# maniac-mc/maniac-mc

Measured on AMD Instinct MI355X. Metric: MC moves/sec, higher is better.
Workload: dtype f64

## Files before the change

### maniac_mc_amd/csrc/mgpu_kernels_pair.h

```cpp
#ifndef MGPU_KERNELS_PAIR_H
#define MGPU_KERNELS_PAIR_H

#include "mgpu_kernels_common.h"

namespace mgpu {

template <int NS, bool ORDERED, bool TRI, bool FUSED, bool FASTW, bool SC1OUT = false>
__device__ __forceinline__ void pair_sweep_item(
    const Topo &tp, const BoxDev &bx, const double *__restrict__ pos, const int *__restrict__ nmol,
    const double *__restrict__ res_q, const int *__restrict__ res_atype, const double2 *__restrict__ pair_tab,
    const char *__restrict__ s_coul, const double2 *__restrict__ s_pair, double *__restrict__ w_site, int *__restrict__ w_sty,
    const PairItem it, const double *__restrict__ cand_sites, int site_stride, int split, int nsplit, int lane,
    double2 *__restrict__ partials, int w) {
    static_assert(!FUSED || (NS > 0 && !ORDERED && !TRI), "the fused old + new sweep is a register-site, unordered, orthorhombic path");
    static_assert(!FASTW || (NS > 0 && !ORDERED && !TRI), "the two-instruction fold is a register-site, unordered, orthorhombic path");
    constexpr int NTY = NS > 0 ? NS : 1;
    constexpr int NST = FUSED ? 2 : 1;
    constexpr int NREG = NTY * NST;
    const int nt = tp.n_types;
    [[maybe_unused]] const char *coul_adj = coul_tab_adjusted(s_coul, bx.coul_idx_base);
    {
        const double *px = pos + (size_t)it.replica * 3 * tp.n_cap_atoms;
        const double *py = px + tp.n_cap_atoms, *pz = py + tp.n_cap_atoms;
        const int *nm_r = nmol + it.replica * tp.n_res;
        const int n1 = NS > 0 ? NS : tp.n1[it.t];
        constexpr bool ordered = ORDERED;

        auto load_site = [&](int a, double &x, double &y, double &z) {
            if (it.src < 0) {
                const int j = atom_slot(tp, it.t, it.m, a);
                x = px[j]; y = py[j]; z = pz[j];
            } else {
                const double *c = cand_sites + ((size_t)it.src * site_stride + a) * 3;
                x = c[0]; y = c[1]; z = c[2];
            }
        };
        double rx[NREG], ry[NREG], rz[NREG], rq[NTY];
        int rty[NTY];
        if constexpr (NS > 0) {
#pragma unroll
            for (int a = 0; a < NTY; ++a) {
                if constexpr (FUSED) {
                    const int j = atom_slot(tp, it.t, it.m, a);
                    rx[a] = px[j]; ry[a] = py[j]; rz[a] = pz[j];
                    const double *c = cand_sites + ((size_t)it.src * site_stride + a) * 3;
                    rx[NTY + a] = c[0]; ry[NTY + a] = c[1]; rz[NTY + a] = c[2];
                    asm volatile("" : "+v"(rx[NTY + a]), "+v"(ry[NTY + a]), "+v"(rz[NTY + a]));
                } else {
                    load_site(a, rx[a], ry[a], rz[a]);
                }
                rq[a] = res_q[it.t * tp.max_atom + a];
                rty[a] = res_atype[it.t * tp.max_atom + a];
                asm volatile("" : "+v"(rx[a]), "+v"(ry[a]), "+v"(rz[a]));
            }
        }

        double elj[NST], ec[NST];
#pragma unroll
        for (int st = 0; st < NST; ++st) { elj[st] = 0.0; ec[st] = 0.0; }
        for (int sb = 0; sb < n1; sb += kSiteChunk) {
            const int ns = NS > 0 ? NS : min(kSiteChunk, n1 - sb);
            if constexpr (NS == 0) {
                __builtin_amdgcn_fence(__ATOMIC_ACQ_REL, "wavefront");
                __builtin_amdgcn_wave_barrier();
                if (lane < ns) {
                    double x, y, z;
                    load_site(sb + lane, x, y, z);
                    w_site[lane * 4 + 0] = x; w_site[lane * 4 + 1] = y; w_site[lane * 4 + 2] = z;
                    w_site[lane * 4 + 3] = res_q[it.t * tp.max_atom + sb + lane];
                    w_sty[lane] = res_atype[it.t * tp.max_atom + sb + lane];
                }
                __builtin_amdgcn_fence(__ATOMIC_ACQ_REL, "wavefront");
                __builtin_amdgcn_wave_barrier();
            }
            for (int t2 = 0, plane_base = 0; t2 < tp.n_res; plane_base += tp.n1[t2], ++t2) {
                if (ordered && t2 < it.t) continue;
                const int nm = nm_r[t2], n2 = tp.n1[t2];
                if (nm == 0) continue;
                const bool same_t = (t2 == it.t) && (it.m >= 0);
                [[maybe_unused]] auto plane_sweep = [&](const double *pxp, const double *pyp, const double *pzp,
                                                        int nm, bool excl, int dummy_m, double qj, int tyj, int key) {
                    const int cpp = (nm + 63) >> 6;
                    const bool qj_on = fabs(qj) >= kErrorTol;
                    double e4[NTY], sg2[NTY], qq[NTY];
                    bool lj[NTY], c_on[NTY];
                    bool any_c = false, all_c = true, any_lj = false;
#pragma unroll
                    for (int s = 0; s < NTY; ++s) {
                        const double2 pt = pair_tab[rty[s] * nt + tyj];
                        e4[s] = pt.x; sg2[s] = pt.y;
                        lj[s] = pt.x != 0.0;
                        c_on[s] = qj_on && (fabs(rq[s]) >= kErrorTol);
                        qq[s] = c_on[s] ? rq[s] * qj : 0.0;
                        any_c = any_c || c_on[s]; all_c = all_c && c_on[s]; any_lj = any_lj || lj[s];
                    }
                    if (!(any_c || any_lj)) return;
                    int c = split - (key * cpp) % nsplit;
                    if (c < 0) c += nsplit;
                    if (c >= cpp) return;
                    auto is_special = [&](int cc) {
                        return ORDERED || (cc == cpp - 1 && (nm & 63) != 0) || (excl && cc == (it.m >> 6));
                    };
                    auto fetch = [&](int cc, bool special, double &x, double &y, double &z, bool &ok) {
                        int m2 = cc * 64 + lane;
                        ok = true;
                        if (special) {
                            asm volatile("" ::: "memory");
                            ok = m2 < nm;
                            if (excl) ok = ok && (ORDERED ? (m2 > it.m) : (m2 != it.m));
                            m2 = ok ? m2 : dummy_m;
                        }
                        const unsigned ob = (unsigned)m2 * 8u;
                        x = *reinterpret_cast<const double *>(reinterpret_cast<const char *>(pxp) + ob);
                        y = *reinterpret_cast<const double *>(reinterpret_cast<const char *>(pyp) + ob);
                        z = *reinterpret_cast<const double *>(reinterpret_cast<const char *>(pzp) + ob);
                    };
                    double acc[NREG];
#pragma unroll
                    for (int s = 0; s < NREG; ++s) acc[s] = 0.0;
                    auto sweep_plane = [&](auto all_tag) {
                        constexpr bool ALL_C = decltype(all_tag)::value;
                        auto unit = [&](double xj, double yj, double zj, double wq, bool valid) {
                            const double rc2l = valid ? bx.rc2 : -1.0;
                            double r2[NREG], g[NREG];
                            unsigned sh_min = ~0u;
                            if constexpr (TRI) {
                                bool ok = bx.tri_lower != 0;
                                if (ok) {
#pragma unroll
                                    for (int s = 0; s < NREG; ++s) ok = image_r2_tri_lower(xj - rx[s], yj - ry[s], zj - rz[s], bx, r2[s]) && ok;
                                }
                                if (!__all(ok)) {
                                    asm volatile("" ::: "memory");
#pragma unroll
                                    for (int s = 0; s < NREG; ++s) r2[s] = image_r2_search27(xj - rx[s], yj - ry[s], zj - rz[s], bx.m);
                                }
                            } else {
#pragma unroll
                                for (int s = 0; s < NREG; ++s) {
                                    r2[s] = FASTW ? image_r2_fast(xj - rx[s], yj - ry[s], zj - rz[s], bx)
                                                  : image_r2<false>(xj - rx[s], yj - ry[s], zj - rz[s], bx);
                                }
                            }
#pragma unroll
                            for (int s = 0; s < NREG; ++s) {
                                if (!ALL_C && !c_on[s % NTY]) { g[s] = 0.0; continue; }
                                unsigned sh;
                                g[s] = coul_lds(r2[s], coul_adj, bx.coul_idx_far, sh);
                                sh_min = min(sh_min, sh);
                            }
                            if (sh_min < (unsigned)bx.coul_idx_base) {
#pragma unroll
                                for (int s = 0; s < NREG; ++s)
                                    if ((ALL_C || c_on[s % NTY]) && r2[s] < kCoulSlowBelow) g[s] = coul_slow(r2[s], bx.alpha, ORDERED);
                            }
#pragma unroll
                            for (int s = 0; s < NREG; ++s)
                                if (ALL_C || c_on[s % NTY]) acc[s] = fma(wq, g[s], acc[s]);
                            if (any_lj) {
#pragma unroll
                                for (int s = 0; s < NREG; ++s) {
                                    if (!lj[s % NTY]) continue;
                                    const double s2 = sg2[s % NTY] * fast_rcp(r2[s]);
                                    const double s6 = s2 * s2 * s2;
                                    const double e = e4[s % NTY] * fma(s6, s6, -s6);
                                    elj[s / NTY] += (r2[s] < rc2l) ? e : 0.0;
                                }
                            }
                        };
                        double xj, yj, zj;
                        bool valid, special = is_special(c);
                        fetch(c, special, xj, yj, zj, valid);
                        for (; c < cpp; c += nsplit) {
                            double xn = xj, yn = yj, zn = zj;
                            bool vn = true;
                            const bool special_n = is_special(c + nsplit);
                            if (c + nsplit < cpp) fetch(c + nsplit, special_n, xn, yn, zn, vn);
                            unit(xj, yj, zj, valid ? 1.0 : 0.0, valid);
                            xj = xn; yj = yn; zj = zn; valid = vn; special = special_n;
                        }
                    };
                    if (all_c) sweep_plane(std::true_type{});
                    else sweep_plane(std::false_type{});
#pragma unroll
                    for (int s = 0; s < NREG; ++s) ec[s / NTY] = fma(qq[s % NTY], acc[s], ec[s / NTY]);
                };
                if (!tp.site_major[t2]) {
                    if constexpr (NS > 0) {
                        const int cap2 = tp.cap[t2], seg2 = tp.seg_off[t2];
                        int dummy_m = 0;
                        if (same_t) {
                            if (ORDERED) { if (it.m + 1 >= nm) continue; dummy_m = nm - 1; }
                            else { if (nm == 1) continue; dummy_m = (it.m == 0) ? 1 : 0; }
                        }
                        for (int a2 = 0; a2 < n2; ++a2) {
                            const double qj = res_q[t2 * tp.max_atom + a2];
                            const int tyj = res_atype[t2 * tp.max_atom + a2];
                            plane_sweep(px + seg2 + a2 * cap2, py + seg2 + a2 * cap2, pz + seg2 + a2 * cap2, nm, same_t, dummy_m, qj, tyj,
                                        plane_base + a2);
                        }
                    } else {
                        const int cpp = (nm + 63) >> 6, units = n2 * cpp;
                        for (int u = split; u < units; u += nsplit) {
                            const int a2 = u / cpp, m2 = (u - a2 * cpp) * 64 + lane;
                            bool valid = m2 < nm;
                            if (same_t) valid = valid && (ordered ? (m2 > it.m) : (m2 != it.m));
                            const double qj = res_q[t2 * tp.max_atom + a2];
                            const int tyj = res_atype[t2 * tp.max_atom + a2];
                            const bool qj_on = fabs(qj) >= kErrorTol;
                            double xj = 0.0, yj = 0.0, zj = 0.0;
                            if (valid) {
                                const int j = tp.seg_off[t2] + a2 * tp.cap[t2] + m2;
                                xj = px[j]; yj = py[j]; zj = pz[j];
                            }
                            for (int s = 0; s < ns; ++s) {
                                const double qs = w_site[s * 4 + 3];
                                const double2 pt = s_pair[w_sty[s] * nt + tyj];
                                const bool do_c = qj_on && (fabs(qs) >= kErrorTol);
                                const bool do_lj = pt.x != 0.0;
                                if ((do_c || do_lj) && valid)
                                    pair_term<ORDERED, TRI>(xj - w_site[s * 4 + 0], yj - w_site[s * 4 + 1], zj - w_site[s * 4 + 2],
                                                       bx, qs * qj, pt.x, pt.y, do_lj, do_c, s_coul, elj[0], ec[0]);
                            }
                        }
                    }
                } else {
                    const int cpp = (n2 + 63) >> 6, units = nm * cpp;
                    for (int u = split; u < units; u += nsplit) {
                        const int m2 = u / cpp, a2 = (u - m2 * cpp) * 64 + lane;
                        if (same_t && (ordered ? (m2 <= it.m) : (m2 == it.m))) continue;
                        const bool valid = a2 < n2;
                        double xj = 0.0, yj = 0.0, zj = 0.0, qj = 0.0;
                        int tyj = 0;
                        if (valid) {
                            const int j = tp.seg_off[t2] + m2 * n2 + a2;
                            xj = px[j]; yj = py[j]; zj = pz[j];
                            qj = res_q[t2 * tp.max_atom + a2];
                            tyj = res_atype[t2 * tp.max_atom + a2];
                        }
                        const bool qj_on = fabs(qj) >= kErrorTol;
                        auto one_site = [&](double sx, double sy, double sz, double qs, int tys, double &elj_s, double &ec_s) {
                            const double2 pt = s_pair[tys * nt + tyj];
                            const bool do_c = qj_on && (fabs(qs) >= kErrorTol);
                            const bool do_lj = pt.x != 0.0;
                            if (valid && (do_lj || do_c))
                                pair_term<ORDERED, TRI, FASTW>(xj - sx, yj - sy, zj - sz, bx, qs * qj, pt.x, pt.y, do_lj, do_c, s_coul, elj_s, ec_s);
                        };
                        if constexpr (NS > 0) {
#pragma unroll
                            for (int s = 0; s < NREG; ++s) one_site(rx[s], ry[s], rz[s], rq[s % NTY], rty[s % NTY], elj[s / NTY], ec[s / NTY]);
                        } else {
                            for (int s = 0; s < ns; ++s)
                                one_site(w_site[s * 4 + 0], w_site[s * 4 + 1], w_site[s * 4 + 2], w_site[s * 4 + 3], w_sty[s], elj[0], ec[0]);
                        }
                    }
                }
            }
        }
#pragma unroll
        for (int st = 0; st < NST; ++st) {
            const double a = wave_sum(elj[st]), b = wave_sum(ec[st]);
            if (lane == 0) store_partial<SC1OUT>(partials + (size_t)w * NST + st, a, b);
        }
    }
}

template <int NS, bool ORDERED, bool TRI, bool FUSED = false, bool FASTW = false>
__global__ __launch_bounds__(kPairBlock, MGPU_PAIR_MINWAVES) void pair_sweep_kernel(
    Topo tp, BoxDev bx, const double *__restrict__ pos, const int *__restrict__ nmol,
    const double *__restrict__ res_q, const int *__restrict__ res_atype, const double2 *__restrict__ pair_tab,
    const char *__restrict__ coul_tab_g, const PairItem *__restrict__ items, const double *__restrict__ cand_sites,
    int site_stride, int nsplit, int n_work, double2 *__restrict__ partials) {
    constexpr int NST = FUSED ? 2 : 1;
    constexpr int NSLAB = NS > 0 ? 1 : kPairWaves * kSiteChunk;
    extern __shared__ __attribute__((aligned(16))) char s_coul[];
    __shared__ double2 s_pair[kMaxTypes * kMaxTypes];
    __shared__ double s_site[NSLAB * 4];
    __shared__ int s_sty[NSLAB];

    for (int i = threadIdx.x; i < (bx.coul_last_row + 1) * kCoulRowVec; i += kPairBlock)
        reinterpret_cast<double2 *>(s_coul)[i] = reinterpret_cast<const double2 *>(coul_tab_g)[i];
    const int nt = tp.n_types;
    for (int i = threadIdx.x; i < nt * nt; i += kPairBlock) s_pair[i] = pair_tab[i];
    __syncthreads();

    const int lane = threadIdx.x & 63;
    const int wave = __builtin_amdgcn_readfirstlane(threadIdx.x >> 6);
    const int n_waves = gridDim.x * kPairWaves;
    double *w_site = s_site + (NS > 0 ? 0 : wave * kSiteChunk * 4);
    int *w_sty = s_sty + (NS > 0 ? 0 : wave * kSiteChunk);

    for (int w = blockIdx.x * kPairWaves + wave; w < n_work; w += n_waves) {
        const int item_id = w / nsplit, split = w - item_id * nsplit;
        const PairItem it = items[item_id];
        pair_sweep_item<NS, ORDERED, TRI, FUSED, FASTW>(tp, bx, pos, nmol, res_q, res_atype, pair_tab, s_coul, s_pair, w_site, w_sty, it,
                                                        cand_sites, site_stride, split, nsplit, lane, partials, w);
    }
}


template <int NS, bool FUSED, bool FASTW, bool SC1OUT = false>
__device__ __forceinline__ void pair_flat_item(
    const Topo &tp, const BoxDev &bx, const double *__restrict__ pos, const int *__restrict__ nmol,
    const double *__restrict__ res_q, const int *__restrict__ res_atype, const char *__restrict__ s_coul,
    const double2 *__restrict__ s_pair, const int4 *__restrict__ s_grp, int4 *__restrict__ w_plane, const PairItem it,
    const double *__restrict__ cand_sites, int site_stride, int split, int nsplit, int lane, int skip_frozen,
    double2 *__restrict__ partials, int w) {
    static_assert(NS > 0, "register sites only");
    constexpr int NTY = NS;
    constexpr int NST = FUSED ? 2 : 1;
    constexpr int NREG = NTY * NST;
    const int nt = tp.n_types;
    const char *coul_adj = coul_tab_adjusted(s_coul, bx.coul_idx_base);
    {
        const double *px = pos + (size_t)it.replica * 3 * tp.n_cap_atoms;
        const double *py = px + tp.n_cap_atoms, *pz = py + tp.n_cap_atoms;
        const int *nm_r = nmol + it.replica * tp.n_res;
        int nmv[kMaxRes];
#pragma unroll
        for (int i = 0; i < kMaxRes; ++i) nmv[i] = i < tp.n_res ? nm_r[i] : 0;

        double rx[NREG], ry[NREG], rz[NREG], rq[NTY];
        int rty[NTY];
#pragma unroll
        for (int a = 0; a < NTY; ++a) {
            if constexpr (FUSED) {
                const int j = atom_slot(tp, it.t, it.m, a);
                rx[a] = px[j]; ry[a] = py[j]; rz[a] = pz[j];
                const double *c = cand_sites + ((size_t)it.src * site_stride + a) * 3;
                rx[NTY + a] = c[0]; ry[NTY + a] = c[1]; rz[NTY + a] = c[2];
            } else if (it.src < 0) {
                const int j = atom_slot(tp, it.t, it.m, a);
                rx[a] = px[j]; ry[a] = py[j]; rz[a] = pz[j];
            } else {
                const double *c = cand_sites + ((size_t)it.src * site_stride + a) * 3;
                rx[a] = c[0]; ry[a] = c[1]; rz[a] = c[2];
            }
            rq[a] = res_q[it.t * tp.max_atom + a];
            rty[a] = res_atype[it.t * tp.max_atom + a] * nt;
        }
#pragma unroll
        for (int k = 0; k < NREG; ++k) asm volatile("" : "+v"(rx[k]), "+v"(ry[k]), "+v"(rz[k]));
        bool any_c = false;
#pragma unroll
        for (int s = 0; s < NTY; ++s) {
            const bool on = fabs(rq[s]) >= kErrorTol;
            any_c = any_c || on;
            rq[s] = on ? rq[s] : 0.0;
        }

        int e_off = 0, e_cnt = 0, e_flags = 0;
        {
            int first = 0;
#pragma unroll
            for (int i = 0; i < kMaxRes; ++i) {
                const int nm2 = nmv[i];
                const bool frozen = tp.site_major[i] == 2;
                const int npl = nm2 == 0 ? 0 : (frozen ? nm2 * tp.n_grp[i] : tp.n1[i]);
                const bool same_t = (i == it.t) && (it.m >= 0);
                const int pl = lane - first;
                if (pl >= 0 && pl < npl) {
                    if (frozen) {
                        const int ng = tp.n_grp[i];
                        const int m2 = nm2 == 1 ? 0 : pl / ng;
                        const int4 gr = s_grp[tp.grp_off[i] + (pl - m2 * ng)];
                        e_off = tp.seg_off[i] + m2 * tp.n1[i] + gr.x;
                        e_cnt = ((same_t && m2 == it.m) || skip_frozen) ? 0 : gr.y;
                        e_flags = 0;
                    } else {
                        e_off = tp.seg_off[i] + pl * tp.cap[i];
                        e_cnt = (same_t && nm2 == 1) ? 0 : nm2;
                        e_flags = same_t ? (1 | ((it.m == 0 ? 1 : 0) << 1)) : 0;
                    }
                }
                first += npl;
            }
        }
        const int e_units = (e_cnt + 63) >> 6;
        int e_incl = e_units;
#pragma unroll
        for (int off = 1; off < 64; off <<= 1) {
            const int v = __shfl_up(e_incl, off, 64);
            e_incl += lane >= off ? v : 0;
        }
        const int n_units = __builtin_amdgcn_readlane(e_incl, 63);
        __builtin_amdgcn_fence(__ATOMIC_ACQ_REL, "wavefront");
        __builtin_amdgcn_wave_barrier();
        w_plane[lane] = make_int4(e_off, e_cnt, e_flags, e_incl - e_units);
        __builtin_amdgcn_fence(__ATOMIC_ACQ_REL, "wavefront");
        __builtin_amdgcn_wave_barrier();
        const int u_begin = (int)(((long long)n_units * split) / nsplit), u_end = (int)(((long long)n_units * (split + 1)) / nsplit);
        int u = u_begin, p = -1, c = 0, cpp = 0;
        int p_off = 0, p_cnt = 0, p_excl = -1, p_dummy = 0;
        bool done = u >= u_end;
        auto load_plane = [&]() {
            const int4 e = w_plane[p];
            p_off = __builtin_amdgcn_readfirstlane(e.x);
            p_cnt = __builtin_amdgcn_readfirstlane(e.y);
            const int fl = __builtin_amdgcn_readfirstlane(e.z);
            const int us = __builtin_amdgcn_readfirstlane(e.w);
            p_excl = (fl & 1) ? it.m : -1;
            p_dummy = fl >> 1;
            cpp = (p_cnt + 63) >> 6;
            c = u - us;
        };
        if (!done) {
            const unsigned long long mk = __ballot(e_units > 0 && (e_incl - e_units) <= u_begin);
            p = 63 - __builtin_clzll(mk);
            load_plane();
        }
        auto next_unit = [&]() {
            ++u;
            ++c;
            if (u >= u_end) { done = true; return; }
            while (c >= cpp) {
                ++p;
                load_plane();
            }
        };
        auto fetch = [&](double &x, double &y, double &z, double &q, int &ty, bool &ok) {
            const int m2 = c * 64 + lane;
            ok = m2 < p_cnt && m2 != p_excl;
            const int j = p_off + (ok ? m2 : p_dummy);
            x = px[j]; y = py[j]; z = pz[j];
            q = tp.slot_q[j];
            ty = tp.slot_ty[j];
        };

        double acc[NREG], elj[NST];
#pragma unroll
        for (int s = 0; s < NREG; ++s) acc[s] = 0.0;
#pragma unroll
        for (int st = 0; st < NST; ++st) elj[st] = 0.0;

        double xn = 0.0, yn = 0.0, zn = 0.0, qn = 0.0;
        int tyn = 0;
        bool vn = false;
        if (!done) fetch(xn, yn, zn, qn, tyn, vn);
        while (!done) {
            const double xj = xn, yj = yn, zj = zn;
            const bool valid = vn;
            const double wq = (valid && fabs(qn) >= kErrorTol) ? qn : 0.0;
            const int tyj = __builtin_amdgcn_readfirstlane(tyn);
            next_unit();
            if (!done) fetch(xn, yn, zn, qn, tyn, vn);

            const double rc2l = valid ? bx.rc2 : -1.0;
            double r2[NREG];
#pragma unroll
            for (int s = 0; s < NREG; ++s)
                r2[s] = FASTW ? image_r2_fast(xj - rx[s], yj - ry[s], zj - rz[s], bx)
                              : image_r2<false>(xj - rx[s], yj - ry[s], zj - rz[s], bx);
            if (any_c && __ballot(wq != 0.0) != 0ull) {
                double g[NREG];
                unsigned sh_min = ~0u;
#pragma unroll
                for (int s = 0; s < NREG; ++s) {
                    unsigned sh;
                    g[s] = coul_lds(r2[s], coul_adj, bx.coul_idx_far, sh);
                    sh_min = min(sh_min, sh);
                }
                if (sh_min < (unsigned)bx.coul_idx_base) {
#pragma unroll
                    for (int s = 0; s < NREG; ++s)
                        if (r2[s] < kCoulSlowBelow) g[s] = coul_slow(r2[s], bx.alpha, false);
                }
#pragma unroll
                for (int s = 0; s < NREG; ++s) acc[s] = fma(wq, g[s], acc[s]);
            }
            double2 pt[NTY];
            bool lj_on[NTY];
#pragma unroll
            for (int s = 0; s < NTY; ++s) pt[s] = s_pair[rty[s] + tyj];
#pragma unroll
            for (int s = 0; s < NTY; ++s)
                lj_on[s] = (__builtin_amdgcn_readfirstlane(__double2hiint(pt[s].x)) | __builtin_amdgcn_readfirstlane(__double2loint(pt[s].x))) != 0;
#pragma unroll
            for (int s = 0; s < NTY; ++s) {
                if (!lj_on[s]) continue;
#pragma unroll
                for (int st = 0; st < NST; ++st) {
                    const double rr = r2[st * NTY + s];
                    const double s2 = pt[s].y * fast_rcp(rr);
                    const double s6 = s2 * s2 * s2;
                    const double e = pt[s].x * fma(s6, s6, -s6);
                    elj[st] += (rr < rc2l) ? e : 0.0;
                }
            }
        }
#pragma unroll
        for (int st = 0; st < NST; ++st) {
            double ec = 0.0;
#pragma unroll
            for (int s = 0; s < NTY; ++s) ec = fma(rq[s], acc[st * NTY + s], ec);
            const double a = wave_sum(elj[st]), b = wave_sum(ec);
            if (lane == 0) store_partial<SC1OUT>(partials + (size_t)w * NST + st, a, b);
        }
    }
}

template <int NS, bool FUSED, bool FASTW>
__global__ __launch_bounds__(kPairBlock, MGPU_PAIR_MINWAVES) void pair_flat_kernel(
    Topo tp, BoxDev bx, const double *__restrict__ pos, const int *__restrict__ nmol,
    const double *__restrict__ res_q, const int *__restrict__ res_atype, const double2 *__restrict__ pair_tab,
    const char *__restrict__ coul_tab_g, const PairItem *__restrict__ items, const double *__restrict__ cand_sites,
    int site_stride, int nsplit, int n_work, double2 *__restrict__ partials, int skip_frozen) {
    constexpr int NST = FUSED ? 2 : 1;
    extern __shared__ __attribute__((aligned(16))) char s_coul[];
    __shared__ double2 s_pair[kMaxTypes * kMaxTypes];
    __shared__ int4 s_grp[kMaxGrp];
    __shared__ int4 s_plane[kPairWaves * kFlatMaxPlanes];

    if (threadIdx.x < kMaxGrp) s_grp[threadIdx.x] = make_int4(tp.grp_start[threadIdx.x], tp.grp_cnt[threadIdx.x], tp.grp_ty[threadIdx.x], 0);
    for (int i = threadIdx.x; i < (bx.coul_last_row + 1) * kCoulRowVec; i += kPairBlock)
        reinterpret_cast<double2 *>(s_coul)[i] = reinterpret_cast<const double2 *>(coul_tab_g)[i];
    const int nt = tp.n_types;
    for (int i = threadIdx.x; i < nt * nt; i += kPairBlock) s_pair[i] = pair_tab[i];
    __syncthreads();

    const int lane = threadIdx.x & 63;
    const int wave = __builtin_amdgcn_readfirstlane(threadIdx.x >> 6);
    const int n_waves = gridDim.x * kPairWaves;

    for (int w = blockIdx.x * kPairWaves + wave; w < n_work; w += n_waves) {
        const int item_id = w / nsplit, split = w - item_id * nsplit;
        const PairItem it = items[item_id];
        pair_flat_item<NS, FUSED, FASTW>(tp, bx, pos, nmol, res_q, res_atype, s_coul, s_pair, s_grp, s_plane + wave * kFlatMaxPlanes, it,
                                         cand_sites, site_stride, split, nsplit, lane, skip_frozen, partials, w);
    }
}


template <int NS, bool FUSED, bool FASTW>
__global__ __launch_bounds__(kPairBlock, MGPU_PAIR_MINWAVES) void pair_frozen_kernel(
    Topo tp, BoxDev bx, const double *__restrict__ pos, const int *__restrict__ nmol,
    const double *__restrict__ res_q, const int *__restrict__ res_atype, const double2 *__restrict__ pair_tab,
    const char *__restrict__ coul_tab_g, const PairItem *__restrict__ items, const double *__restrict__ cand_sites,
    int site_stride, int n_items, int t_frozen, int n_chunks, int chunk_atoms, double2 *__restrict__ scratch,
    int *__restrict__ tickets, double2 *__restrict__ extra, const double *__restrict__ slot_q_on, const int *__restrict__ slot_ty) {
    constexpr int NTY = NS;
    constexpr int NST = FUSED ? 2 : 1;
    constexpr int NREG = NTY * NST;
    extern __shared__ __attribute__((aligned(16))) char s_coul[];
    __shared__ double2 s_pair[kMaxTypes * kMaxTypes];
    __shared__ double s_cand[NREG * 3 * 64];
    __shared__ double2 s_part[kPairWaves * NST * 64];
    __shared__ int s_last;
    for (int i = threadIdx.x; i < (bx.coul_last_row + 1) * kCoulRowVec; i += kPairBlock)
        reinterpret_cast<double2 *>(s_coul)[i] = reinterpret_cast<const double2 *>(coul_tab_g)[i];
    const int nt = tp.n_types;
    for (int i = threadIdx.x; i < nt * nt; i += kPairBlock) s_pair[i] = pair_tab[i];
    __syncthreads();

    const int lane = threadIdx.x & 63;
    const int wave = __builtin_amdgcn_readfirstlane(threadIdx.x >> 6);
    const char *coul_adj = coul_tab_adjusted(s_coul, bx.coul_idx_base);
    const int n_groups = (n_items + 63) >> 6;
    const int n_atoms = nmol[t_frozen] * tp.n1[t_frozen];
    const double *fx = pos + tp.seg_off[t_frozen], *fy = fx + tp.n_cap_atoms, *fz = fy + tp.n_cap_atoms;
    const double *__restrict__ fq = slot_q_on + tp.seg_off[t_frozen];
    const int *__restrict__ fty = slot_ty + tp.seg_off[t_frozen];

    const int wg_per_group = (n_chunks + kPairWaves - 1) / kPairWaves;
    const int n_wg_units = n_groups * wg_per_group;
    for (int b = blockIdx.x; b < n_wg_units; b += gridDim.x) {
        const int grp = b / wg_per_group, chunk = (b - grp * wg_per_group) * kPairWaves + wave;
        __syncthreads();
        for (int idx = threadIdx.x; idx < NREG * 3 * 64; idx += kPairBlock) {
            const int ln = idx & 63, comp = idx >> 6, sreg = comp / 3, d = comp - 3 * sreg;
            const int id = grp * 64 + ln;
            const PairItem il = items[id < n_items ? id : n_items - 1];
            const double *pd = pos + (size_t)il.replica * 3 * tp.n_cap_atoms + (size_t)d * tp.n_cap_atoms;
            const bool resident = FUSED ? (sreg < NTY) : (il.src < 0);
            const int a = (FUSED && sreg >= NTY) ? sreg - NTY : sreg;
            s_cand[idx] = resident ? pd[atom_slot(tp, il.t, il.m, a)]
                                   : cand_sites[((size_t)(il.src < 0 ? 0 : il.src) * site_stride + a) * 3 + d];
        }
        __syncthreads();
        do {
        if (chunk >= n_chunks) break;
        const int item_id = grp * 64 + lane;
        const bool live = item_id < n_items;
        const PairItem it = items[live ? item_id : n_items - 1];
        const double *px = pos + (size_t)it.replica * 3 * tp.n_cap_atoms;
        const double *py = px + tp.n_cap_atoms, *pz = py + tp.n_cap_atoms;
        double rx[NREG], ry[NREG], rz[NREG], rq[NTY];
        int rty[NTY];
#pragma unroll
        for (int sreg = 0; sreg < NREG; ++sreg) {
            rx[sreg] = s_cand[(sreg * 3 + 0) * 64 + lane];
            ry[sreg] = s_cand[(sreg * 3 + 1) * 64 + lane];
            rz[sreg] = s_cand[(sreg * 3 + 2) * 64 + lane];
        }
        const int t_item = __builtin_amdgcn_readfirstlane(it.t);
        bool any_c = false, q_on[NTY];
#pragma unroll
        for (int s = 0; s < NTY; ++s) {
            rq[s] = res_q[t_item * tp.max_atom + s];
            rty[s] = res_atype[t_item * tp.max_atom + s] * nt;
            q_on[s] = fabs(rq[s]) >= kErrorTol;
            any_c = any_c || q_on[s];
            rq[s] = q_on[s] ? rq[s] : 0.0;
        }
        const int a0 = chunk * chunk_atoms, na = min(chunk_atoms, n_atoms - a0);

        double acc[NREG], elj[NST];
#pragma unroll
        for (int s = 0; s < NREG; ++s) acc[s] = 0.0;
#pragma unroll
        for (int st = 0; st < NST; ++st) elj[st] = 0.0;
        int cur_ty = -1;
        double e4[NTY], sg2[NTY];
        bool lj_on[NTY];
#pragma unroll
        for (int s = 0; s < NTY; ++s) { e4[s] = 0.0; sg2[s] = 0.0; lj_on[s] = false; }
        for (int k = 0; k < na; ++k) {
            const int jk = __builtin_amdgcn_readfirstlane(a0 + k);
            const double xj = fx[jk], yj = fy[jk], zj = fz[jk];
            const double qj = fq[jk];
            const int tyj = fty[jk];
            if (tyj != cur_ty) {
                cur_ty = tyj;
#pragma unroll
                for (int s = 0; s < NTY; ++s) {
                    const double2 pt = s_pair[rty[s] + tyj];
                    e4[s] = __hiloint2double(__builtin_amdgcn_readfirstlane(__double2hiint(pt.x)), __builtin_amdgcn_readfirstlane(__double2loint(pt.x)));
                    sg2[s] = __hiloint2double(__builtin_amdgcn_readfirstlane(__double2hiint(pt.y)), __builtin_amdgcn_readfirstlane(__double2loint(pt.y)));
                    lj_on[s] = e4[s] != 0.0;
                }
            }
            double r2[NREG];
#pragma unroll
            for (int s = 0; s < NREG; ++s)
                r2[s] = FASTW ? image_r2_fast(xj - rx[s], yj - ry[s], zj - rz[s], bx)
                              : image_r2<false>(xj - rx[s], yj - ry[s], zj - rz[s], bx);
            if (any_c && qj != 0.0) {
                double g[NREG];
                unsigned sh_min = ~0u;
#pragma unroll
                for (int s = 0; s < NREG; ++s) {
                    g[s] = 0.0;
                    if (q_on[s % NTY]) {
                        unsigned sh;
                        g[s] = coul_lds(r2[s], coul_adj, bx.coul_idx_far, sh);
                        sh_min = min(sh_min, sh);
                    }
                }
                if (sh_min < (unsigned)bx.coul_idx_base) {
#pragma unroll
                    for (int s = 0; s < NREG; ++s)
                        if (q_on[s % NTY] && r2[s] < kCoulSlowBelow) g[s] = coul_slow(r2[s], bx.alpha, false);
                }
#pragma unroll
                for (int s = 0; s < NREG; ++s) acc[s] = fma(qj, g[s], acc[s]);
            }
#pragma unroll
            for (int s = 0; s < NTY; ++s) {
                if (!lj_on[s]) continue;
#pragma unroll
                for (int st = 0; st < NST; ++st) {
                    const double rr = r2[st * NTY + s];
                    const double s2 = sg2[s] * fast_rcp(rr);
                    const double s6 = s2 * s2 * s2;
                    const double e = e4[s] * fma(s6, s6, -s6);
                    elj[st] += (rr < bx.rc2) ? e : 0.0;
                }
            }
        }
        for (int t2 = 0; t2 < tp.n_res; ++t2) {
            if (tp.site_major[t2] != 0) continue;
            const int nm_l = live ? nmol[it.replica * tp.n_res + t2] : 0;
            int nm_max = nm_l;
#pragma unroll
            for (int off = 32; off > 0; off >>= 1) nm_max = max(nm_max, __shfl_xor(nm_max, off, 64));
            nm_max = __builtin_amdgcn_readfirstlane(nm_max);
            const int n2 = tp.n1[t2], cap2 = tp.cap[t2], seg2 = tp.seg_off[t2];
            const bool same_t = t2 == t_item;
            for (int m2 = chunk; m2 < nm_max; m2 += n_chunks) {
                const bool ok = m2 < nm_l && !(same_t && m2 == it.m);
                for (int a2 = 0; a2 < n2; ++a2) {
                    double qj = res_q[t2 * tp.max_atom + a2];
                    qj = fabs(qj) >= kErrorTol ? qj : 0.0;
                    const int tyj = res_atype[t2 * tp.max_atom + a2];
                    const int j = seg2 + a2 * cap2 + (ok ? m2 : 0);
                    const double xj = px[j], yj = py[j], zj = pz[j];
                    double r2[NREG];
#pragma unroll
                    for (int s = 0; s < NREG; ++s)
                        r2[s] = FASTW ? image_r2_fast(xj - rx[s], yj - ry[s], zj - rz[s], bx)
                                      : image_r2<false>(xj - rx[s], yj - ry[s], zj - rz[s], bx);
                    if (any_c && qj != 0.0) {
                        double g[NREG];
                        unsigned sh_min = ~0u;
#pragma unroll
                        for (int s = 0; s < NREG; ++s) {
                            g[s] = 0.0;
                            if (q_on[s % NTY]) {
                                unsigned sh;
                                g[s] = coul_lds(r2[s], coul_adj, bx.coul_idx_far, sh);
                                sh_min = min(sh_min, sh);
                            }
                        }
                        if (ok && sh_min < (unsigned)bx.coul_idx_base) {
#pragma unroll
                            for (int s = 0; s < NREG; ++s)
                                if (ok && q_on[s % NTY] && r2[s] < kCoulSlowBelow) g[s] = coul_slow(r2[s], bx.alpha, false);
                        }
#pragma unroll
                        for (int s = 0; s < NREG; ++s) acc[s] = ok ? fma(qj, g[s], acc[s]) : acc[s];
                    }
#pragma unroll
                    for (int s = 0; s < NTY; ++s) {
                        const double2 pt = pair_tab[rty[s] + tyj];
                        if (pt.x == 0.0) continue;
#pragma unroll
                        for (int st = 0; st < NST; ++st) {
                            const double rr = r2[st * NTY + s];
                            const double s2 = pt.y * fast_rcp(rr);
                            const double s6 = s2 * s2 * s2;
                            const double e = pt.x * fma(s6, s6, -s6);
                            elj[st] += (ok && rr < bx.rc2) ? e : 0.0;
                        }
                    }
                }
            }
        }
#pragma unroll
        for (int st = 0; st < NST; ++st) {
            double ec = 0.0;
#pragma unroll
            for (int s = 0; s < NTY; ++s) ec = fma(rq[s], acc[st * NTY + s], ec);
            s_part[(wave * NST + st) * 64 + lane] = make_double2(elj[st], ec);
        }
        } while (0);
        __syncthreads();
        const int wgc = b - grp * wg_per_group;
        const int st_t = threadIdx.x >> 6, id_t = grp * 64 + lane;
        const bool summing = (int)threadIdx.x < NST * 64 && id_t < n_items;
        double2 *rec = scratch + ((size_t)id_t * NST + st_t);
        if (summing) {
            const int n_valid = min(kPairWaves, n_chunks - wgc * kPairWaves);
            double ea = 0.0, eb = 0.0;
            for (int wv = 0; wv < n_valid; ++wv) {
                const double2 pp = s_part[(wv * NST + st_t) * 64 + lane];
                ea += pp.x; eb += pp.y;
            }
            store_partial<true>(rec + (size_t)wgc * ((size_t)n_items * NST), ea, eb);
        }
        asm volatile("s_waitcnt vmcnt(0)" ::: "memory");
        __syncthreads();
        if (threadIdx.x == 0) s_last = atomicAdd(&tickets[grp], 1) == wg_per_group - 1;
        __syncthreads();
        if (s_last) {
            if (summing) {
                double ea = 0.0, eb = 0.0;
                for (int q = 0; q < wg_per_group; ++q) {
                    const double *pr = reinterpret_cast<const double *>(rec + (size_t)q * ((size_t)n_items * NST));
                    ea += load_sc1(pr); eb += load_sc1(pr + 1);
                }
                extra[(size_t)id_t * NST + st_t] = make_double2(ea, eb);
            }
            if (threadIdx.x == 0) __hip_atomic_store(&tickets[grp], 0, __ATOMIC_RELAXED, __HIP_MEMORY_SCOPE_AGENT);
        }
    }
}

static __global__ void pair_finalize_kernel(const double2 *__restrict__ partials, int n_items, int nsplit,
                                     double *__restrict__ e_lj, double *__restrict__ e_coul) {
    const int i = blockIdx.x * blockDim.x + threadIdx.x;
    if (i >= n_items) return;
    double a = 0.0, b = 0.0;
    for (int s = 0; s < nsplit; ++s) { const double2 p = partials[(size_t)i * nsplit + s]; a += p.x; b += p.y; }
    e_lj[i] = a;
    e_coul[i] = b * kEps0InvEvA / kKbEvK;
}

}

#endif
```

Baseline: 8.408 million.

## Add scalar-register uniform pair sweep path for three-site fused fast kernels

Adds a specialised pair sweep for the fused, fast-fold, three-site case. It reads kernel arguments directly through the kernarg constant address space and loads site coordinates with one lane-parallel fetch, then broadcasts them into scalar registers with readlane. The aim is to move wave-uniform values (sites, charges, flags, box parameters) out of vector registers and into SGPRs, cutting VGPR pressure and redundant per-lane loads. It also prefetches the next chunk inside the plane loop. It relies on reinterpreting the kernarg segment as a struct layout that must match the kernel signature, and it adds a lot of inline-asm register constraints.

```diff
diff --git a/maniac_mc_amd/csrc/mgpu_kernels_pair.h b/maniac_mc_amd/csrc/mgpu_kernels_pair.h
--- a/maniac_mc_amd/csrc/mgpu_kernels_pair.h
+++ b/maniac_mc_amd/csrc/mgpu_kernels_pair.h
@@ -265,6 +265,245 @@
     }
 }
 
+struct PairSweepArgs {
+    Topo tp;
+    BoxDev bx;
+    const double *pos;
+    const int *nmol;
+    const double *res_q;
+    const int *res_atype;
+    const double2 *pair_tab;
+    const char *coul_tab_g;
+    const PairItem *items;
+    const double *cand_sites;
+    int site_stride, nsplit, n_work;
+    double2 *partials;
+};
+#define MGPU_KCONST __attribute__((address_space(4)))
+template <class T>
+__device__ __forceinline__ const MGPU_KCONST T *launch_const(const T *p) { return (const MGPU_KCONST T *)p; }
+__device__ __forceinline__ PairItem load_item(const MGPU_KCONST PairItem *p) {
+    PairItem it;
+    it.replica = p->replica; it.t = p->t; it.m = p->m; it.src = p->src; it.ordered = p->ordered;
+    return it;
+}
+__device__ __forceinline__ double wave_uniform(double v) {
+    return __hiloint2double(__builtin_amdgcn_readfirstlane(__double2hiint(v)), __builtin_amdgcn_readfirstlane(__double2loint(v)));
+}
+
+__device__ __forceinline__ int uniform_flag(bool b) {
+    int f = __builtin_amdgcn_readfirstlane(b ? 1 : 0);
+    asm volatile("" : "+s"(f));
+    return f;
+}
+
+template <int NS>
+__device__ __forceinline__ void pair_sweep_item_uniform(const MGPU_KCONST PairSweepArgs *ka, const char *__restrict__ s_coul,
+                                                        const double2 *__restrict__ s_pair, int lane, int w) {
+    constexpr int NTY = NS, NST = 2, NREG = NTY * NST;
+    int site_pack = 0;
+    {
+        const MGPU_KCONST PairSweepArgs &k = *ka;
+        const MGPU_KCONST Topo &tp = k.tp;
+        const int item_id = w / k.nsplit;
+        const PairItem it = load_item(launch_const(k.items) + item_id);
+        const int i = min(lane >> 1, 3 * NREG - 1), sreg = i / 3, d = i - 3 * sreg, a = sreg < NTY ? sreg : sreg - NTY;
+        const int j = tp.site_major[it.t] ? tp.seg_off[it.t] + it.m * tp.n1[it.t] + a : tp.seg_off[it.t] + a * tp.cap[it.t] + it.m;
+        const double *src = sreg < NTY ? k.pos + ((size_t)it.replica * 3 + d) * tp.n_cap_atoms + j
+                                       : k.cand_sites + ((size_t)it.src * k.site_stride + a) * 3 + d;
+        site_pack = reinterpret_cast<const int *>(src)[lane & 1];
+    }
+    double rx[NREG], ry[NREG], rz[NREG];
+    auto unpack_sites = [&]() {
+        auto coord = [&](int i) {
+            double v = __hiloint2double(__builtin_amdgcn_readlane(site_pack, 2 * i + 1), __builtin_amdgcn_readlane(site_pack, 2 * i));
+            asm volatile("" : "+s"(v));
+            return v;
+        };
+#pragma unroll
+        for (int s = 0; s < NREG; ++s) { rx[s] = coord(3 * s); ry[s] = coord(3 * s + 1); rz[s] = coord(3 * s + 2); }
+    };
+    double elj[NST], ec[NST];
+#pragma unroll
+    for (int st = 0; st < NST; ++st) { elj[st] = 0.0; ec[st] = 0.0; }
+    int t2 = 0, a2 = 0, plane_base = 0;
+    for (;;) {
+        asm volatile("" : "+s"(ka));
+        const MGPU_KCONST PairSweepArgs &k = *ka;
+        const MGPU_KCONST Topo &tp = k.tp;
+        if (t2 >= tp.n_res) break;
+        BoxDev bx;
+#pragma unroll
+        for (int d = 0; d < 3; ++d) bx.L[d] = k.bx.L[d];
+        bx.rc2 = k.bx.rc2; bx.alpha = k.bx.alpha;
+        bx.coul_idx_base = k.bx.coul_idx_base; bx.coul_idx_far = k.bx.coul_idx_far; bx.coul_idx_end = k.bx.coul_idx_end;
+        const int nt = tp.n_types, nsplit = k.nsplit, item_id = w / nsplit, split = w - item_id * nsplit;
+        const PairItem it = load_item(launch_const(k.items) + item_id);
+        const int nm = launch_const(k.nmol)[it.replica * tp.n_res + t2], n2 = tp.n1[t2];
+        const bool same_t = (t2 == it.t) && (it.m >= 0);
+        const bool plane_major = !tp.site_major[t2];
+        if (nm == 0 || (plane_major && same_t && nm == 1)) { plane_base += n2; ++t2; a2 = 0; continue; }
+        const MGPU_KCONST double *px = launch_const(k.pos) + (size_t)it.replica * 3 * tp.n_cap_atoms;
+        const MGPU_KCONST double *py = px + tp.n_cap_atoms, *pz = py + tp.n_cap_atoms;
+        const char *coul_adj = coul_tab_adjusted(s_coul, bx.coul_idx_base);
+        double rq[NTY];
+        int rty[NTY];
+#pragma unroll
+        for (int a = 0; a < NTY; ++a) {
+            rq[a] = launch_const(k.res_q)[it.t * tp.max_atom + a];
+            rty[a] = launch_const(k.res_atype)[it.t * tp.max_atom + a];
+        }
+        if (plane_major) {
+            const int cap2 = tp.cap[t2], seg2 = tp.seg_off[t2];
+            const int dummy_m = (same_t && it.m == 0) ? 1 : 0;
+            const bool excl = same_t;
+            const double qj = launch_const(k.res_q)[t2 * tp.max_atom + a2];
+            const int tyj = launch_const(k.res_atype)[t2 * tp.max_atom + a2];
+            const int key = plane_base + a2;
+            const double *pxp = (const double *)(px + seg2 + a2 * cap2), *pyp = (const double *)(py + seg2 + a2 * cap2),
+                         *pzp = (const double *)(pz + seg2 + a2 * cap2);
+            if (++a2 == n2) { plane_base += n2; ++t2; a2 = 0; }
+            const int cpp = (nm + 63) >> 6;
+            const bool qj_on = fabs(qj) >= kErrorTol;
+            double e4[NTY], sg2[NTY], qq[NTY];
+            bool lj[NTY], c_on[NTY];
+            bool any_c = false, all_c = true, any_lj = false;
+#pragma unroll
+            for (int s = 0; s < NTY; ++s) {
+                const MGPU_KCONST double *pt = reinterpret_cast<const MGPU_KCONST double *>(launch_const(k.pair_tab) + (rty[s] * nt + tyj));
+                e4[s] = pt[0]; sg2[s] = pt[1];
+                lj[s] = e4[s] != 0.0;
+                c_on[s] = qj_on && (fabs(rq[s]) >= kErrorTol);
+                qq[s] = c_on[s] ? rq[s] * qj : 0.0;
+                any_c = any_c || c_on[s]; all_c = all_c && c_on[s]; any_lj = any_lj || lj[s];
+            }
+            if (!(any_c || any_lj)) continue;
+#pragma unroll
+            for (int s = 0; s < NTY; ++s) { qq[s] = wave_uniform(qq[s]); asm volatile("" : "+s"(qq[s])); }
+            int on = 0;
+#pragma unroll
+            for (int s = 0; s < NTY; ++s) on |= (lj[s] ? 1 << s : 0) | (c_on[s] ? 0x100 << s : 0);
+            on = __builtin_amdgcn_readfirstlane(on);
+            asm volatile("" : "+s"(on));
+            const int lj_any = uniform_flag(any_lj);
+            int c = split - (key * cpp) % nsplit;
+            if (c < 0) c += nsplit;
+            if (c >= cpp) continue;
+            auto is_special = [&](int cc) { return uniform_flag((cc == cpp - 1 && (nm & 63) != 0) || (excl && cc == (it.m >> 6))); };
+            auto fetch = [&](int cc, int special, double &x, double &y, double &z, bool &ok) {
+                int m2 = cc * 64 + lane;
+                ok = true;
+                if (special) {
+                    asm volatile("" ::: "memory");
+                    ok = m2 < nm;
+                    if (excl) ok = ok && (m2 != it.m);
+                    m2 = ok ? m2 : dummy_m;
+                }
+                const unsigned ob = (unsigned)m2 * 8u;
+                x = *reinterpret_cast<const double *>(reinterpret_cast<const char *>(pxp) + ob);
+                y = *reinterpret_cast<const double *>(reinterpret_cast<const char *>(pyp) + ob);
+                z = *reinterpret_cast<const double *>(reinterpret_cast<const char *>(pzp) + ob);
+            };
+            double acc[NREG];
+#pragma unroll
+            for (int s = 0; s < NREG; ++s) acc[s] = 0.0;
+            auto sweep_plane = [&](auto all_tag) {
+                constexpr bool ALL_C = decltype(all_tag)::value;
+                unpack_sites();
+                auto unit = [&](double xj, double yj, double zj, double wq, double rc2l) {
+                    asm volatile("" : "+s"(on));
+                    double r2[NREG], g[NREG];
+                    unsigned sh_min = ~0u;
+#pragma unroll
+                    for (int s = 0; s < NREG; ++s) r2[s] = image_r2_fast(xj - rx[s], yj - ry[s], zj - rz[s], bx);
+#pragma unroll
+                    for (int s = 0; s < NREG; ++s) {
+                        if (!ALL_C && !(on & (0x100 << (s % NTY)))) { g[s] = 0.0; continue; }
+                        unsigned sh;
+                        g[s] = coul_lds(r2[s], coul_adj, bx.coul_idx_far, sh);
+                        sh_min = min(sh_min, sh);
+                    }
+                    if (__builtin_expect(sh_min < (unsigned)bx.coul_idx_base, 0)) {
+#pragma unroll
+                        for (int s = 0; s < NREG; ++s)
+                            if ((ALL_C || (on & (0x100 << (s % NTY)))) && r2[s] < kCoulSlowBelow) g[s] = coul_slow(r2[s], k.bx.alpha, false);
+                    }
+#pragma unroll
+                    for (int s = 0; s < NREG; ++s)
+                        if (ALL_C || (on & (0x100 << (s % NTY)))) acc[s] = fma(wq, g[s], acc[s]);
+                    if (lj_any) {
+#pragma unroll
+                        for (int s = 0; s < NREG; ++s) {
+                            if (!(on & (1 << (s % NTY)))) continue;
+                            const double s2 = sg2[s % NTY] * fast_rcp(r2[s]);
+                            const double s6 = s2 * s2 * s2;
+                            const double e = e4[s % NTY] * fma(s6, s6, -s6);
+                            elj[s / NTY] += (r2[s] < rc2l) ? e : 0.0;
+                        }
+                    }
+                };
+                auto masks = [&](bool ok, double &wq, double &rc2l) {
+                    wq = ok ? 1.0 : 0.0;
+                    rc2l = ok ? bx.rc2 : -1.0;
+                    asm volatile("" : "+v"(wq), "+v"(rc2l));
+                };
+                double xj, yj, zj, wq, rc2l;
+                bool valid;
+                fetch(c, is_special(c), xj, yj, zj, valid);
+                masks(valid, wq, rc2l);
+                for (; c < cpp; c += nsplit) {
+                    double xn = xj, yn = yj, zn = zj, wn = wq, rn = rc2l;
+                    if (c + nsplit < cpp) {
+                        bool vn;
+                        fetch(c + nsplit, is_special(c + nsplit), xn, yn, zn, vn);
+                        masks(vn, wn, rn);
+                    }
+                    unit(xj, yj, zj, wq, rc2l);
+                    xj = xn; yj = yn; zj = zn; wq = wn; rc2l = rn;
+                }
+            };
+            if (all_c) sweep_plane(std::true_type{});
+            else sweep_plane(std::false_type{});
+#pragma unroll
+            for (int s = 0; s < NREG; ++s) ec[s / NTY] = fma(qq[s % NTY], acc[s], ec[s / NTY]);
+        } else {
+            const int cpp = (n2 + 63) >> 6, units = nm * cpp;
+            unpack_sites();
+            for (int u = split; u < units; u += nsplit) {
+                const int m2 = u / cpp, sa = (u - m2 * cpp) * 64 + lane;
+                if (same_t && m2 == it.m) continue;
+                const bool valid = sa < n2;
+                double xj = 0.0, yj = 0.0, zj = 0.0, qj = 0.0;
+                int tyj = 0;
+                if (valid) {
+                    const int j = tp.seg_off[t2] + m2 * n2 + sa;
+                    xj = px[j]; yj = py[j]; zj = pz[j];
+                    qj = launch_const(k.res_q)[t2 * tp.max_atom + sa];
+                    tyj = launch_const(k.res_atype)[t2 * tp.max_atom + sa];
+                }
+                const bool qj_on = fabs(qj) >= kErrorTol;
+#pragma unroll
+                for (int s = 0; s < NREG; ++s) {
+                    const double2 pt = s_pair[rty[s % NTY] * nt + tyj];
+                    const bool do_c = qj_on && (fabs(rq[s % NTY]) >= kErrorTol);
+                    const bool do_lj = pt.x != 0.0;
+                    if (valid && (do_lj || do_c))
+                        pair_term<false, false, true>(xj - rx[s], yj - ry[s], zj - rz[s], bx, rq[s % NTY] * qj, pt.x, pt.y, do_lj, do_c, s_coul,
+                                                      elj[s / NTY], ec[s / NTY]);
+                }
+            }
+            plane_base += n2; ++t2; a2 = 0;
+        }
+    }
+#pragma unroll
+    for (int st = 0; st < NST; ++st) {
+        const double a = wave_sum(elj[st]), b = wave_sum(ec[st]);
+        if (lane == 0) store_partial<false>(ka->partials + (size_t)w * NST + st, a, b);
+    }
+}
+
+template <int NS> constexpr bool kPairUniformSites = NS == 3;
+
 template <int NS, bool ORDERED, bool TRI, bool FUSED = false, bool FASTW = false>
 __global__ __launch_bounds__(kPairBlock, MGPU_PAIR_MINWAVES) void pair_sweep_kernel(
     Topo tp, BoxDev bx, const double *__restrict__ pos, const int *__restrict__ nmol,
@@ -290,6 +529,12 @@
     double *w_site = s_site + (NS > 0 ? 0 : wave * kSiteChunk * 4);
     int *w_sty = s_sty + (NS > 0 ? 0 : wave * kSiteChunk);
 
+    if constexpr (FUSED && FASTW && kPairUniformSites<NS>) {
+        const auto *ka = (const MGPU_KCONST PairSweepArgs *)__builtin_amdgcn_kernarg_segment_ptr();
+        for (int w = blockIdx.x * kPairWaves + wave; w < ka->n_work; w += gridDim.x * kPairWaves)
+            pair_sweep_item_uniform<NS>(ka, s_coul, s_pair, lane, w);
+        return;
+    }
     for (int w = blockIdx.x * kPairWaves + wave; w < n_work; w += n_waves) {
         const int item_id = w / nsplit, split = w - item_id * nsplit;
         const PairItem it = items[item_id];
```

After: 8.436 million (median of 4 runs). About the same (+0.3%).
